# lyndonchan/wsss-analysis

Measured on AMD Instinct MI355X. Metric: images/sec CAM+CRF pseudo-labels, VOC2012 321x321, higher is better.
Workload: dtype f16x3; 1 GPU; resnet50 CAM + dense-CRF (M=21, 10 mean-field iters), 321x321, batch 32 images (=64 samples) per GPU, image-sharded; batch_images=32, num_classes=20, parallelism=image-sharded x1, no collective, steps_per_rank=239

## Files before the change

include/wsscam.h:

```cpp
#ifndef WSSCAM_H
#define WSSCAM_H

#include <stddef.h>
#include <stdint.h>

#ifdef __cplusplus
extern "C" {
#endif

#define WSC_VERSION 100

typedef enum wsc_status {
    WSC_OK = 0,
    WSC_ERR_INVALID = -1,
    WSC_ERR_NO_DEVICE = -2,
    WSC_ERR_HIP = -3,
    WSC_ERR_MISSING_KEY = -4,
    WSC_ERR_SHAPE = -5,
    WSC_ERR_NOMEM = -6,
    WSC_ERR_KEY_RANGE = -7,
    WSC_ERR_CAPACITY = -8,
    WSC_ERR_RANGE = -9
} wsc_status;

typedef enum wsc_arch {
    WSC_ARCH_RESNET50_CAM = 0,
    WSC_ARCH_VGG16_CAM = 1,
    WSC_ARCH_M7_CAM = 2,
    WSC_ARCH_RESNET50_IRN = 3,
    WSC_ARCH_VGG16_IRN = 4,
    WSC_ARCH_M7_IRN = 5,
    WSC_ARCH_DEEPLAB_LFOV = 6,
    WSC_ARCH_DEEPLAB_ASPP = 7
} wsc_arch;

typedef enum wsc_precision {
    WSC_PREC_BF16 = 0,
    WSC_PREC_BF16X3 = 1,
    WSC_PREC_F16 = 2,
    WSC_PREC_F16X3 = 3,
    WSC_PREC_F32 = 4
} wsc_precision;

typedef struct wsc_ctx wsc_ctx;
typedef struct wsc_net wsc_net;
typedef enum {
    WSC_OPT_CRF_GAUSS_ON_CHIP = 0,
    WSC_OPT_CRF_FUSED_BLUR = 1,
    WSC_OPT_CRF_BLUR_ON_CHIP = 2,
    WSC_OPT_CRF_RANK_BALLOT = 3,
    WSC_OPT_CRF_EMBED_FULL = 4,
    WSC_OPT_RW_TILED = 5,
    WSC_OPT_STEM_POOL_FUSED = 6,
    WSC_OPT_CONV_WINDOW = 7,
    WSC_OPT_CAM_HEAD_STREAM = 8,
    WSC_OPT_CRF_MSG_IN_UPDATE = 9,
    WSC_OPT_COUNT = 10
} wsc_option;

typedef struct wsc_crf wsc_crf;
typedef struct wsc_crf_v wsc_crf_v;

typedef struct wsc_tensor_desc {
    const char *name;
    const float *data;
    int32_t ndim;
    int64_t shape[4];
} wsc_tensor_desc;


int wsc_version(void);
const char *wsc_last_error(void);

int wsc_ctx_create(int device, void *stream, wsc_ctx **out);
void wsc_ctx_destroy(wsc_ctx *ctx);
int wsc_ctx_set_option(wsc_ctx *ctx, int option, int value);
int wsc_sync(wsc_ctx *ctx);
int wsc_ctx_range_status(wsc_ctx *ctx, int *flag_out, int clear);
int wsc_ctx_wait(wsc_ctx *ctx, wsc_ctx *other);
int wsc_ctx_mark(wsc_ctx *ctx, int slot);
int wsc_ctx_wait_mark(wsc_ctx *ctx, int slot);
int wsc_ctx_wait_for_mark(wsc_ctx *ctx, wsc_ctx *other, int slot);
int wsc_device_info(wsc_ctx *ctx, char *arch_name, size_t arch_name_len, int *num_cus);

int wsc_malloc(wsc_ctx *ctx, size_t bytes, void **dptr_out);
int wsc_free(wsc_ctx *ctx, void *dptr);
int wsc_memcpy_h2d(wsc_ctx *ctx, void *dst_dev, const void *src_host, size_t bytes);
int wsc_memcpy_d2h(wsc_ctx *ctx, void *dst_host, const void *src_dev, size_t bytes);
int wsc_memset(wsc_ctx *ctx, void *dst_dev, int value, size_t bytes);
int wsc_host_alloc(wsc_ctx *ctx, size_t bytes, void **host_out);
// ... 319 lines not shown
```

wsss-analysis_amd/csrc/common.h:

```cpp
#pragma once
#include <hip/hip_runtime.h>
#include <assert.h>
#include <stdint.h>
#include <map>
#include <string>
#include <unordered_map>
#include <vector>

#include "../../include/wsscam.h"

typedef uint16_t bf16_t;

typedef __bf16 bf16x8_t __attribute__((ext_vector_type(8)));
typedef _Float16 f16x8_t __attribute__((ext_vector_type(8)));
typedef float f32x16_t __attribute__((ext_vector_type(16)));
typedef float f32x4_t __attribute__((ext_vector_type(4)));

__host__ __device__ inline bf16_t f32_to_bf16(float f) {
    union { float f; uint32_t u; } v;
    v.f = f;
    uint32_t u = v.u;
    if ((u & 0x7fffffffu) > 0x7f800000u) return (bf16_t)((u >> 16) | 0x40);
    u += 0x7fffu + ((u >> 16) & 1u);
    return (bf16_t)(u >> 16);
// ... 85 lines not shown
    WSC_K_SLICE_UPDATE,
    WSC_K_CRF_MISC,
    WSC_K_WGRAD,
    WSC_K_GRAD_MISC,
    WSC_K_UPSAMPLE_GRAD,
    WSC_K_GN_GRAD,
    WSC_K_COUNT
};
struct WscProfRecord {
    int cls;
    double work;
    hipEvent_t e0, e1;
};

struct WscGaussCache;
void wsc_gauss_cache_destroy(WscGaussCache *cache);
struct wsc_ctx {
    int device = 0;
    hipStream_t stream = nullptr;
    bool own_stream = false;
    int num_cus = 0;
    std::string arch;
    void *ws = nullptr;
    size_t ws_bytes = 0;
    static constexpr int PIN_SLOTS = 8;
    struct PinSlot {
        void *p = nullptr;
        size_t bytes = 0;
        hipEvent_t ev = nullptr;
        bool busy = false;
    };
    PinSlot pin_ring[PIN_SLOTS];
    int pin_next = 0;
    int opt[WSC_OPT_COUNT] = {1, 1, 1, 0, 0, -1, 1, 1, 1, 1};
    void *zero_page = nullptr;
    unsigned *range_host = nullptr, *range_dev = nullptr;
    hipEvent_t ev0 = nullptr, ev1 = nullptr;
    hipEvent_t join_ev = nullptr;
    hipEvent_t marks[8] = {};
    bool mark_set[8] = {};
    hipStream_t aux_stream = nullptr;
    hipEvent_t fork_ev = nullptr, aux_done_ev = nullptr;
    bool profiling = false;
    std::vector<WscProfRecord> prof;
    std::vector<hipEvent_t> prof_pool;
    std::multimap<size_t, void *> free_blocks;
    std::unordered_map<void *, size_t> live_blocks;
    WscGaussCache *gauss_cache = nullptr;
};
int wsc_ctx_workspace(wsc_ctx *ctx, size_t bytes, void **out);
int wsc_ctx_range_check(wsc_ctx *ctx);
__device__ __forceinline__ unsigned half2_at_ceiling(unsigned hw) { return (hw & 0x7fff7fffu) + 0x04010401u; }
struct WscKernelTimer {
    wsc_ctx *ctx;
    int idx = -1;
    WscKernelTimer(wsc_ctx *c, int cls, double work);
    ~WscKernelTimer();
};
int wsc_ctx_cached_alloc(wsc_ctx *ctx, size_t bytes, void **out);
void wsc_ctx_cached_free(wsc_ctx *ctx, void *p);
struct WscCachedGuard {
    wsc_ctx *ctx;
    void *p;
    WscCachedGuard(wsc_ctx *c, void *q) : ctx(c), p(q) {}
    WscCachedGuard(const WscCachedGuard &) = delete;
    WscCachedGuard &operator=(const WscCachedGuard &) = delete;
    void free_now() {
// ... 334 lines not shown
```

wsss-analysis_amd/csrc/conv_igemm.hip:

```cpp
#include "common.h"

#include <type_traits>

namespace {

constexpr int BK = 64;

struct ConvKArgs {
    const bf16_t *x, *x_lo, *w;
    const float *s1, *b1, *s2, *b2;
    const bf16_t *res, *res_lo;
    bf16_t *y, *y_lo;
    float *y_f32;
    int H, W, Cin, Ho, Wo, Cout;
    int ldy;
    int kh, kw, stride, pad, relu;
    int M, HoWo;
    int m_base, m_end;
    unsigned div_howo_mul, div_howo_s1, div_howo_s2, div_wo_mul, div_wo_s1, div_wo_s2;
    int cchunks;
    int dil;
    int ksteps_base;
    int nk;
    int Kw;
    int Kbase;
    int ntiles_n, nblocks;
    const bf16_t *zero;
    int spare1;
    long long lo_delta;
    const bf16_t *x2;
    long long lo_delta2;
    int cc2, H2, W2, C2, stride2;
    int ldx;
    int win_npix;
    int spare2, spare3;
    unsigned *range;
};

__device__ __forceinline__ int lds_off(int row, int slot) {
    return row * 128 + ((slot ^ ((row >> 1) & 7)) << 4);
}

__device__ __forceinline__ void decode_row(const ConvKArgs &p, int m, int &n, int &ho, int &wo) {
    const unsigned t1 = __umulhi(p.div_howo_mul, (unsigned)m);
    n = (int)((t1 + (((unsigned)m - t1) >> p.div_howo_s1)) >> p.div_howo_s2);
    const int rem = m - n * p.HoWo;
    const unsigned t2 = __umulhi(p.div_wo_mul, (unsigned)rem);
    ho = (int)((t2 + (((unsigned)rem - t2) >> p.div_wo_s1)) >> p.div_wo_s2);
    wo = rem - ho * p.Wo;
}

template <int BM, int BN, int MODE, int SPLIT, int ET, int STAGES, int FAST = 0, int WPT = 0>
__global__ __launch_bounds__(BM * 2, (STAGES == 1 && FAST != 0) ? 4 : 2) void conv_igemm_kernel(ConvKArgs p) {
    constexpr bool GLDS = MODE == 0;
    constexpr int WMT = BM == 256 ? 128 : 64;
    constexpr bool FEPI = (FAST & 1) != 0, PW = (FAST & 2) != 0;
    constexpr bool WIN = WPT > 0;
    static_assert(!WIN || (SPLIT == 2 && BM == 128 && STAGES == 2 && FAST == 1), "LDS window: single-staged split, 128-row tile");
    static_assert(FAST == 0 || (SPLIT != 1 && ET == 1 && (MODE == 0 || FAST == 1)),
                  "FAST paths: f16, one plane or the single-staged split; the pointwise prologue belongs to the LDS-DMA layers");
    static_assert(SPLIT != 2 || (MODE == 0 && STAGES == 2), "single-staged split: LDS-DMA layers, two LDS buffers");
    static_assert(STAGES == 2 || SPLIT == 0, "one LDS buffer serves a one-K-step layer, which a layer of three K segments never is");
    constexpr int CK = SPLIT == 2 ? 32 : 64;
    constexpr int NT = BM * 2;
    constexpr int NW = BM / 32;
    constexpr int WR = BM / WMT;
    constexpr int WC = NW / WR;
    constexpr int WN = BN / WC;
    constexpr int MI = WMT / 32;
    constexpr int NI = WN / 32;
    static_assert(WR * WC == NW && WN % 32 == 0, "wave layout");
    constexpr int NB = BN * 8 / NT;
    constexpr int A_BYTES = BM * BK * 2;
    constexpr int B_BYTES = BN * BK * 2;
    constexpr int WIN_BYTES = WPT * 4096;
    constexpr int A_REGION = WIN ? WIN_BYTES : STAGES * A_BYTES;
    constexpr int CT_STRIDE = BN + 4;
    static_assert(GLDS || (BM == 128 && STAGES <= 2), "register staging exists for the 128-row tile only");
    static_assert(STAGES >= 1 && STAGES <= 2, "1 (single K-step layers) or 2 LDS buffers");

    extern __shared__ __attribute__((aligned(16))) char smem[];

    const int t = threadIdx.x;
    const int lane = t & 63;
    const int wv = __builtin_amdgcn_readfirstlane(t >> 6);
    const int wm = wv / WC, wn = wv - wm * WC;

    int tile;
    {
        const int bid = blockIdx.x;
// ... 103 lines not shown
                                                        c, 0, 0, 0);
        else
            c = __builtin_amdgcn_mfma_f32_32x32x16_f16(__builtin_bit_cast(f16x8_t, a), __builtin_bit_cast(f16x8_t, b),
                                                       c, 0, 0, 0);
    };
    auto mfma0 = [&](const u32x4_t &a, const u32x4_t &b) -> f32x16_t {
        const f32x16_t z = {0.f, 0.f, 0.f, 0.f, 0.f, 0.f, 0.f, 0.f, 0.f, 0.f, 0.f, 0.f, 0.f, 0.f, 0.f, 0.f};
        if (ET == 0)
            return __builtin_amdgcn_mfma_f32_32x32x16_bf16(__builtin_bit_cast(bf16x8_t, a), __builtin_bit_cast(bf16x8_t, b), z, 0, 0, 0);
        return __builtin_amdgcn_mfma_f32_32x32x16_f16(__builtin_bit_cast(f16x8_t, a), __builtin_bit_cast(f16x8_t, b), z, 0, 0, 0);
    };
    const unsigned lds0 = (unsigned)(uintptr_t)(__attribute__((address_space(3))) char *)smem;

    auto compute = [&](int buf) {
        const char *sa = smem + buf * A_BYTES;
        const char *sb = smem + STAGES * A_BYTES + buf * B_BYTES;
#pragma unroll
        for (int ks = 0; ks < 4; ++ks) {
            const int sl = ks * 2 + kgrp;
            u32x4_t af[MI], bfr[NI];
#pragma unroll
            for (int mi = 0; mi < MI; ++mi)
                af[mi] = *reinterpret_cast<const u32x4_t *>(sa + lds_off(wm * WMT + mi * 32 + l31, sl));
#pragma unroll
            for (int ni = 0; ni < NI; ++ni)
                bfr[ni] = *reinterpret_cast<const u32x4_t *>(sb + lds_off(wn * WN + ni * 32 + l31, sl));
#pragma unroll
            for (int mi = 0; mi < MI; ++mi)
#pragma unroll
                for (int ni = 0; ni < NI; ++ni) mfma(af[mi], bfr[ni], acc[mi][ni]);
        }
    };

    const int nk = STAGES == 1 ? 1 : p.nk;
    if (GLDS) {
        int n_seg = 0, n_khi = 0, n_kwi = 0, n_cc = 0, n_ktl = 0;
        const bf16_t *n_src = p.x;
        long long n_tap = 0;
        int n_wk = 0;
        auto prep = [&]() {
            n_src = (SPLIT == 1 && n_seg == 1) ? p.x_lo : p.x;
            if constexpr (FAST == 0) n_tap = ((long long)(n_khi * p.dil) * p.W + n_kwi * p.dil) * p.ldx + n_cc * CK;
            else n_tap = ((long long)n_khi * p.W + n_kwi) * p.ldx + n_cc * CK;
            if (SPLIT != 1 && p.x2 != nullptr && n_cc >= p.cc2) {
                n_src = p.x2;
                n_tap = (n_cc - p.cc2) * CK;
            }
            n_wk = ((SPLIT == 1 && n_seg == 2) ? p.Kbase : 0) + n_ktl * 64;
        };
        auto second_source = [&]() {
#pragma unroll
            for (int i = 0; i < 4; ++i) {
                const int m = m0 + lrow + RSTEP * i;
                int n, ho, wo;
                decode_row(p, m < p.m_end ? m : p.m_end - 1, n, ho, wo);
                const long long b2 = (((long long)n * p.H2 + ho * p.stride2) * p.W2 + wo * p.stride2) * (long long)p.C2;
                const int r = lrow + RSTEP * i;
                const int ks = slot ^ ((r >> 1) & 7);
                if (SPLIT == 2) aoff[i] = b2 + (ks & 3) * 8 + ((ks & 4) ? p.lo_delta2 : 0ll);
                else aoff[i] = b2 + ks * 8;
            }
        };
        auto advance = [&]() {
            ++n_ktl;
            if (++n_kwi == p.kw) {
                n_kwi = 0;
// ... 66 lines not shown
                const long long e = (long long)u * (long long)p.ldx + (sl & 3) * 8 + ((sl & 4) ? p.lo_delta : 0ll);
                woff[i] = ok ? (int)(e >> 3) : 0;
                wvalid |= ok ? (1u << i) : 0u;
            }
            win_load(0);
        }
        prep();
        if constexpr (!WIN) {
#pragma unroll
            for (int i = 0; i < 4; ++i) issue_a(i, 0);
        }
#pragma unroll
        for (int i = 0; i < NB; ++i) issue_b(i, 0);
        advance();
        if constexpr (WIN) win_store();
        if (ROLL && nk > 1) {
            prep();
#pragma unroll
            for (int i = 0; i < 4; ++i) issue_a(i, 1);
#pragma unroll
            for (int i = 0; i < NB; ++i) issue_b(i, 1);
            advance();
            asm volatile("s_waitcnt vmcnt(%0)" ::"n"(4 + NB) : "memory");
            __builtin_amdgcn_s_barrier();
        } else {
            __syncthreads();
        }
        unsigned offA[4], offB[4];
#pragma unroll
        for (int ks = 0; ks < 4; ++ks) {
            offA[ks] = lds0 + lds_off(wm * WMT + l31, ks * 2 + kgrp);
            offB[ks] = lds0 + A_REGION + lds_off(wn * WN + l31, ks * 2 + kgrp);
        }
        auto kstep = [&](auto cur_c, int kt) __attribute__((always_inline)) {
            constexpr int cur = decltype(cur_c)::value;
            const unsigned(&oA)[4] = offA, (&oB)[4] = offB;
            const bool more = kt + 1 < nk;
            if (more) {
                prep();
                if (SPLIT != 2) {
#pragma unroll
                    for (int i = 0; i < 4; ++i) issue_a(i, cur ^ 1);
#pragma unroll
                    for (int i = 0; i < NB; ++i) issue_b(i, cur ^ 1);
                }
            }
            if constexpr (SPLIT == 2) {
                u32x4_t fah[2][MI], fal[2][MI], fbh[2][NI], fbl[2][NI];
                constexpr int NAP = WIN ? 0 : 4;
                constexpr int EVERY = (6 * MI * NI) / (NAP + NB);
                static_assert(EVERY >= 1, "a K-step has room for every DMA piece");
                auto piece = [&](int j) {
                    if (!more || j % EVERY != 0) return;
                    const int q = j / EVERY;
                    if (q < NAP) issue_a(q, cur ^ 1);
                    else if (q < NAP + NB) issue_b(q - NAP, cur ^ 1);
                    __builtin_amdgcn_sched_barrier(0);
                };
                unsigned aw[MI][4];
                if constexpr (WIN) {
                    if ((c_khi | c_kwi) == 0 && c_cc + 1 < p.cchunks) win_load(c_cc + 1);
                    const int toff = c_khi * p.W + c_kwi;
                    const unsigned tbit = 1u << (c_khi * 3 + c_kwi);
#pragma unroll
                    for (int mi = 0; mi < MI; ++mi) {
                        const int pos = (tapmask[mi] & tbit) ? WIN_ZERO : qm[mi] + toff;
                        const unsigned b0 = lds0 + (unsigned)pos * 128u, sw = (unsigned)(pos >> 1) & 7u;
#pragma unroll
                        for (int pr = 0; pr < 4; ++pr) aw[mi][pr] = b0 + ((((unsigned)(pr * 2 + kgrp)) ^ sw) << 4);
                    }
                }
                auto rd = [&](int set, int sl) {
#pragma unroll
                    for (int mi = 0; mi < MI; ++mi) {
                        if constexpr (WIN) {
                            asm volatile("ds_read_b128 %0, %1" : "=v"(fah[set][mi]) : "v"(aw[mi][sl]) : "memory");
                            asm volatile("ds_read_b128 %0, %1" : "=v"(fal[set][mi]) : "v"(aw[mi][2 + sl]) : "memory");
                        } else {
                            asm volatile("ds_read_b128 %0, %1 offset:%2" : "=v"(fah[set][mi]) : "v"(oA[sl]), "n"(cur * A_BYTES + mi * 4096) : "memory");
                            asm volatile("ds_read_b128 %0, %1 offset:%2" : "=v"(fal[set][mi]) : "v"(oA[2 + sl]), "n"(cur * A_BYTES + mi * 4096) : "memory");
                        }
                    }
#pragma unroll
                    for (int ni = 0; ni < NI; ++ni) {
                        asm volatile("ds_read_b128 %0, %1 offset:%2" : "=v"(fbh[set][ni]) : "v"(oB[sl]), "n"(cur * B_BYTES + ni * 4096) : "memory");
                        asm volatile("ds_read_b128 %0, %1 offset:%2" : "=v"(fbl[set][ni]) : "v"(oB[2 + sl]), "n"(cur * B_BYTES + ni * 4096) : "memory");
                    }
                };
                rd(0, 0);
// ... 30 lines not shown
                }
            } else {
                u32x4_t fa[2][MI], fb[2][NI];

                auto rd = [&](int set, int ks) {
#pragma unroll
                    for (int mi = 0; mi < MI; ++mi)
                        asm volatile("ds_read_b128 %0, %1 offset:%2" : "=v"(fa[set][mi]) : "v"(oA[ks]), "n"(cur * A_BYTES + mi * 4096) : "memory");
#pragma unroll
                    for (int ni = 0; ni < NI; ++ni)
                        asm volatile("ds_read_b128 %0, %1 offset:%2" : "=v"(fb[set][ni]) : "v"(oB[ks]), "n"(cur * B_BYTES + ni * 4096) : "memory");
                };
                rd(0, 0);
#pragma unroll
                for (int ks = 0; ks < 4; ++ks) {
                    const int set = ks & 1;
                    if (ks < 3) {
                        rd(set ^ 1, ks + 1);
                        asm volatile("s_waitcnt lgkmcnt(%0)" ::"n"(MI + NI) : "memory");
                    } else {
                        asm volatile("s_waitcnt lgkmcnt(0)" ::: "memory");
                    }
                    __builtin_amdgcn_sched_barrier(0);
#pragma unroll
                    for (int mi = 0; mi < MI; ++mi)
#pragma unroll
                        for (int ni = 0; ni < NI; ++ni) {
                            if (STAGES == 1 && ks == 0) acc[mi][ni] = mfma0(fa[set][mi], fb[set][ni]);
                            else mfma(fa[set][mi], fb[set][ni], acc[mi][ni]);
                        }
                }
            }
            if (more) advance();
            __syncthreads();
            if constexpr (WIN) {
                if (++c_kwi == p.kw) {
                    c_kwi = 0;
                    if (++c_khi == p.kh) {
                        c_khi = 0;
                        ++c_cc;
                        if (more) {
                            win_store();
                            __syncthreads();
                        }
                    }
                }
            }
        };
        static_assert(A_BYTES + (MI - 1) * 4096 < 65536 && B_BYTES + (NI - 1) * 4096 < 65536, "ds_read immediate offset range");
        if constexpr (ROLL) {
            u32x4_t fah[MI], fal[MI], fbh[NI], fbl[NI];
            auto slice = [&](auto buf_c, auto pair_c, bool more, bool dma, int dbuf) __attribute__((always_inline)) {
                constexpr int nbuf = decltype(buf_c)::value, npair = decltype(pair_c)::value;
                const unsigned(&oA)[4] = offA, (&oB)[4] = offB;
                auto piece = [&](int j) {
                    if (!dma || j % 3 != 0) return;
                    const int q = j / 3;
                    if (q < 4) issue_a(q, dbuf);
                    else if (q < 4 + NB) issue_b(q - 4, dbuf);
                    __builtin_amdgcn_sched_barrier(0);
                };
                static_assert(3 * MI * NI >= 3 * (4 + NB), "a slice has room for every DMA piece");
                auto rdA = [&](u32x4_t(&f)[MI], int pair) {
#pragma unroll
                    for (int mi = 0; mi < MI; ++mi)
                        asm volatile("ds_read_b128 %0, %1 offset:%2" : "=v"(f[mi]) : "v"(oA[pair]), "n"(nbuf * A_BYTES + mi * 4096) : "memory");
                };
// ... 36 lines not shown
                        piece(2 * MI * NI + mi * NI + ni);
                    }
                __builtin_amdgcn_sched_barrier(0);
                if (more) {
                    rdB(fbh, npair);
                    rdA(fah, npair);
                }
            };
            {
                const unsigned(&oA)[4] = offA, (&oB)[4] = offB;
#pragma unroll
                for (int mi = 0; mi < MI; ++mi) asm volatile("ds_read_b128 %0, %1 offset:%2" : "=v"(fal[mi]) : "v"(oA[2]), "n"(mi * 4096) : "memory");
#pragma unroll
                for (int ni = 0; ni < NI; ++ni) asm volatile("ds_read_b128 %0, %1 offset:%2" : "=v"(fbl[ni]) : "v"(oB[2]), "n"(ni * 4096) : "memory");
#pragma unroll
                for (int ni = 0; ni < NI; ++ni) asm volatile("ds_read_b128 %0, %1 offset:%2" : "=v"(fbh[ni]) : "v"(oB[0]), "n"(ni * 4096) : "memory");
#pragma unroll
                for (int mi = 0; mi < MI; ++mi) asm volatile("ds_read_b128 %0, %1 offset:%2" : "=v"(fah[mi]) : "v"(oA[0]), "n"(mi * 4096) : "memory");
            }
            auto rstep = [&](auto cur_c, int kt) __attribute__((always_inline)) {
                constexpr int cur = decltype(cur_c)::value;
                slice(std::integral_constant<int, cur>{}, std::integral_constant<int, 1>{}, true, false, 0);
                __syncthreads();
                const bool refill = kt + 2 < nk;
                if (refill) prep();
                slice(std::integral_constant<int, cur ^ 1>{}, std::integral_constant<int, 0>{}, kt + 1 < nk, refill, cur);
                if (refill) advance();
            };
            for (int kt = 0; kt < nk; kt += 2) {
                rstep(std::integral_constant<int, 0>{}, kt);
                if (kt + 1 < nk) rstep(std::integral_constant<int, 1>{}, kt + 1);
            }
            __syncthreads();
        } else
        for (int kt = 0; kt < nk; kt += 2) {
            kstep(std::integral_constant<int, 0>{}, kt);
            if (kt + 1 < nk) kstep(std::integral_constant<int, 1>{}, kt + 1);
        }
    } else {
        load_tile(0);
        store_lds(0);
        __syncthreads();
        for (int kt = 0; kt < nk; ++kt) {
            const int cur = kt & 1;
            const bool more = kt + 1 < nk;
            if (more) load_tile(kt + 1);
            compute(cur);
            if (more) store_lds(cur ^ 1);
            __syncthreads();
        }
    }

    constexpr int TPR = BN / 8;
    constexpr int RPP = NT / TPR;
    constexpr int NPASS = BM / RPP;
    const int c8 = t % TPR;
    const int r0 = t / TPR;
    const int c = n0 + c8 * 8;
    const bool cok = c < p.Cout;
    const bool full = c + 8 <= p.Cout;
    const bool has_res = p.res != nullptr && full;
    constexpr bool PRE_ALL = WMT == 64 && !(STAGES == 1 && FEPI);
    constexpr int NHALF_R = STAGES == 1 ? BM / 64 : (WMT == 128 ? BM / 128 : 1);
    constexpr int NRES = PRE_ALL ? NPASS : NPASS / NHALF_R;
    uint4 rres[NRES], rres_lo[NRES];
    auto fetch_res = [&](int first_pass) {
#pragma unroll
        for (int i = 0; i < NRES; ++i) {
            const int m = m0 + (first_pass + i) * RPP + r0;
            rres[i] = make_uint4(0, 0, 0, 0);
            rres_lo[i] = make_uint4(0, 0, 0, 0);
            if (FEPI) {
                if (has_res) {
                    const int mc = m < p.m_end ? m : p.m_end - 1;
                    rres[i] = *reinterpret_cast<const uint4 *>(p.res + ((unsigned)mc * (unsigned)p.Cout + (unsigned)c));
                    if (SPLIT) rres_lo[i] = *reinterpret_cast<const uint4 *>(p.res_lo + ((unsigned)mc * (unsigned)p.Cout + (unsigned)c));
                }
            } else if (has_res && m < p.m_end) {
                const long long o = (long long)m * p.Cout + c;
                rres[i] = *reinterpret_cast<const uint4 *>(p.res + o);
                if (SPLIT) rres_lo[i] = *reinterpret_cast<const uint4 *>(p.res_lo + o);
            }
        }
    };
    if (PRE_ALL) fetch_res(0);
    const bool fpost = FEPI && p.s2 != nullptr;
    const float sat_lo = (p.relu && !fpost) ? 0.f : -65504.f;
    float s1[8], b1[8], s2[FEPI ? 1 : 8], b2[FEPI ? 1 : 8];
    const bool post = !FEPI && p.s2 != nullptr;
    if (FEPI) {
        const f32x4_t sa = *reinterpret_cast<const f32x4_t *>(p.s1 + c), sb = *reinterpret_cast<const f32x4_t *>(p.s1 + c + 4);
        const f32x4_t ba = *reinterpret_cast<const f32x4_t *>(p.b1 + c), bb = *reinterpret_cast<const f32x4_t *>(p.b1 + c + 4);
#pragma unroll
        for (int j = 0; j < 4; ++j) {
            s1[j] = sa[j];
            s1[4 + j] = sb[j];
            b1[j] = ba[j];
            b1[4 + j] = bb[j];
        }
    } else {
#pragma unroll
        for (int j = 0; j < 8; ++j) {
            s1[j] = cok ? p.s1[c + j] : 0.f;
            b1[j] = cok ? p.b1[c + j] : 0.f;
            s2[j] = (cok && post) ? p.s2[c + j] : 1.f;
            b2[j] = (cok && post) ? p.b2[c + j] : 0.f;
        }
    }

    float *ct = reinterpret_cast<float *>(smem);
    constexpr int NHALF = STAGES == 1 ? BM / 64 : (WMT == 128 ? BM / 128 : 1);
    constexpr int GR = BM / NHALF;
    constexpr int PPH = NPASS / NHALF;
    static_assert(NPASS % NHALF == 0 && PPH * RPP == GR && GR % WMT == 0, "epilogue pass layout");
    const int grp = (wm * WMT) / GR, roff = wm * WMT - grp * GR;
    unsigned ovf = 0u;
#pragma unroll
    for (int half = 0; half < NHALF; ++half) {
        if (half > 0) __syncthreads();
        if (!PRE_ALL) fetch_res(half * PPH);
        if (grp == half) {
#pragma unroll
            for (int mi = 0; mi < MI; ++mi)
#pragma unroll
                for (int ni = 0; ni < NI; ++ni)
#pragma unroll
                    for (int r = 0; r < 16; ++r) {
                        const int row = roff + mi * 32 + (r & 3) + 8 * (r >> 2) + 4 * kgrp;
                        const int col = wn * WN + ni * 32 + l31;
                        ct[row * CT_STRIDE + col] = acc[mi][ni][r];
                    }
        }
        __syncthreads();
        if (!cok) continue;
#pragma unroll
        for (int pp = 0; pp < PPH; ++pp) {
            const int pass = half * PPH + pp;
            const int lrow_e = pp * RPP + r0;
            const int m = m0 + half * GR + lrow_e;
            if (FEPI) {
// ... 99 lines not shown
                }
                if (p.y != nullptr && full) {
                    uint32_t hw[4], lw[4];
#pragma unroll
                    for (int j = 0; j < 4; ++j) {
                        const bf16_t h0 = f32_to_h16(v[2 * j], ET), h1 = f32_to_h16(v[2 * j + 1], ET);
                        hw[j] = (uint32_t)h0 | ((uint32_t)h1 << 16);
                        if (SPLIT) {
                            const float c0 = ET ? fminf(fmaxf(v[2 * j], -65504.f), 65504.f) : v[2 * j];
                            const float c1 = ET ? fminf(fmaxf(v[2 * j + 1], -65504.f), 65504.f) : v[2 * j + 1];
                            const bf16_t l0 = f32_to_h16(c0 - h16_to_f32(h0, ET), ET);
                            const bf16_t l1 = f32_to_h16(c1 - h16_to_f32(h1, ET), ET);
                            lw[j] = (uint32_t)l0 | ((uint32_t)l1 << 16);
                        }
                    }
                    if (ET) ovf |= half2_at_ceiling(hw[0]) | half2_at_ceiling(hw[1]) | half2_at_ceiling(hw[2]) | half2_at_ceiling(hw[3]);
                    const long long oy = (long long)m * p.ldy + c;
                    *reinterpret_cast<uint4 *>(p.y + oy) = make_uint4(hw[0], hw[1], hw[2], hw[3]);
                    if (SPLIT) *reinterpret_cast<uint4 *>(p.y_lo + oy) = make_uint4(lw[0], lw[1], lw[2], lw[3]);
                }
            }
        }
    }
    if (ET && (ovf & 0x80008000u)) *p.range = (unsigned)p.Cout;
}

typedef void (*ConvKernel)(ConvKArgs);
struct ConvVariant {
    ConvKernel kernel;
    int bm, bn;
    int lds;
    int cls;
};
template <int BM, int BN, int MODE, int SPLIT, int ET, int STAGES, int FAST = 0, int WPT = 0>
ConvVariant variant() {
    constexpr int A_BYTES = BM * BK * 2, B_BYTES = BN * BK * 2;
    constexpr int PIPE = WPT > 0 ? WPT * 4096 + STAGES * B_BYTES : STAGES * (A_BYTES + B_BYTES);
    constexpr int EPI = (STAGES == 1 ? 64 : (BM == 256 ? 128 : BM)) * (BN + 4) * 4;
    constexpr int LDS = PIPE > EPI ? PIPE : EPI;
    static_assert(LDS <= 160 * 1024, "LDS budget of a CU");
    return {conv_igemm_kernel<BM, BN, MODE, SPLIT, ET, STAGES, FAST, WPT>, BM, BN, LDS,
            MODE != 0 ? WSC_K_CONV_SMALLCIN : (BM == 256 ? WSC_K_CONV256 : (BN == 128 ? WSC_K_CONV128 : WSC_K_CONV64))};
}
template <int BM, int BN, int MODE, int ET, int FAST = 0>
ConvVariant one_plane(bool one_kstep) {
    if constexpr (BM == 128)
        if (one_kstep) return variant<BM, BN, MODE, 0, ET, 1, FAST>();
    return variant<BM, BN, MODE, 0, ET, 2, FAST>();
}
template <int BM, int BN>
ConvVariant select_variant(ConvForm form, wsc_precision prec, int fast, bool one_kstep, int wpt) {
    if constexpr (BM == 128) {
        auto small = [&](auto mode) {
            constexpr int MODE = decltype(mode)::value;
            switch (prec) {
            case WSC_PREC_BF16: return one_plane<128, BN, MODE, 0>(one_kstep);
            case WSC_PREC_BF16X3: return variant<128, BN, MODE, 1, 0, 2>();
            case WSC_PREC_F16: return fast ? one_plane<128, BN, MODE, 1, 1>(one_kstep) : one_plane<128, BN, MODE, 1>(one_kstep);
            default: return variant<128, BN, MODE, 1, 1, 2>();
            }
        };
        if (form == CONV_FORM_SMALL2) return small(std::integral_constant<int, 1>{});
        if (form == CONV_FORM_SMALL4) return small(std::integral_constant<int, 2>{});
        if (wpt == 8) return variant<128, BN, 0, 2, 1, 2, 1, 8>();
        if (wpt == 10) return variant<128, BN, 0, 2, 1, 2, 1, 10>();
    }
    ConvVariant v;
    switch (prec) {
    case WSC_PREC_BF16: v = one_plane<BM, BN, 0, 0>(one_kstep); break;
    case WSC_PREC_BF16X3: v = variant<BM, BN, 0, 1, 0, 2>(); break;
    case WSC_PREC_F16:
        v = fast == 3 ? one_plane<BM, BN, 0, 1, 3>(one_kstep) : (fast ? one_plane<BM, BN, 0, 1, 1>(one_kstep) : one_plane<BM, BN, 0, 1>(one_kstep));
        break;
    default:
        v = fast == 3 ? variant<BM, BN, 0, 2, 1, 2, 3>() : (fast ? variant<BM, BN, 0, 2, 1, 2, 1>() : variant<BM, BN, 0, 2, 1, 2>());
        break;
    }
    if (form == CONV_FORM_STEM_ROWS) v.cls = WSC_K_CONV_SMALLCIN;
    return v;
}
ConvVariant conv_variant(int bm, int bn, ConvForm form, wsc_precision prec, int fast, bool one_kstep, int wpt = 0) {
    if (bm == 256) return select_variant<256, 256>(form, prec, fast, one_kstep, wpt);
    return bn == 128 ? select_variant<128, 128>(form, prec, fast, one_kstep, wpt) : select_variant<128, 64>(form, prec, fast, one_kstep, wpt);
}

}

int conv_igemm_launch(wsc_ctx *ctx, const ConvLaunch &p) {
    if (p.prec == WSC_PREC_F32) return conv_f32_launch(ctx, p);
    WSC_CHECK(p.operands_match(), WSC_ERR_INVALID, "conv: an operand is not of the layer's precision %d", (int)p.prec);
    const int split = conv_split(p.prec), fmt = conv_fmt(p.prec);
    const bool dma = conv_form_dma(p.form);
    if (p.form == CONV_FORM_STEM_ROWS)
        WSC_CHECK(split == 2 && p.Cin == 4 && p.pad == 0 && p.kw <= 7 && (p.stride & 1) == 0, WSC_ERR_INVALID,
                  "conv: the padded-stem form needs split 2, a 4-channel padded input, kw <= 7 and an even stride");
    else if (p.form == CONV_FORM_GENERIC) WSC_CHECK(p.Cin % 64 == 0, WSC_ERR_INVALID, "conv: Cin=%d not a multiple of 64", p.Cin);
    else WSC_CHECK(p.Cin == 4, WSC_ERR_INVALID, "conv: small-Cin mode needs a 4-channel activation");
    const ConvKLayout k = conv_k_layout(p.kh, p.kw, p.Cin, p.form, p.prec);
    const bool single_staged = k.interleaved;
    ConvKArgs a = {};
    a.x = p.x.h16(); a.x_lo = p.x.h16_lo(); a.w = (const bf16_t *)p.w;
    a.s1 = p.s1; a.b1 = p.b1; a.s2 = p.s2; a.b2 = p.b2;
    a.res = p.res.h16(); a.res_lo = p.res.h16_lo();
    a.y = p.y.h16(); a.y_lo = p.y.h16_lo(); a.y_f32 = p.y_f32;
    a.H = p.H; a.W = p.W; a.Cin = p.Cin; a.Ho = p.Ho; a.Wo = p.Wo; a.Cout = p.Cout;
    a.ldy = p.ldy > 0 ? p.ldy : p.Cout;
    a.win_npix = 0;
    a.ldx = p.Cin; a.x2 = nullptr; a.lo_delta2 = 0; a.cc2 = 0; a.H2 = a.W2 = a.C2 = 0; a.stride2 = 1;
    a.kh = p.kh; a.kw = k.kw_steps; a.stride = p.stride; a.pad = p.pad; a.relu = p.relu;
    a.M = p.N * p.Ho * p.Wo;
    a.HoWo = p.Ho * p.Wo;
    conv_fastdiv((unsigned)(a.HoWo > 0 ? a.HoWo : 1), &a.div_howo_mul, &a.div_howo_s1, &a.div_howo_s2);
    conv_fastdiv((unsigned)(p.Wo > 0 ? p.Wo : 1), &a.div_wo_mul, &a.div_wo_s1, &a.div_wo_s2);
    WSC_CHECK(p.dil >= 1, WSC_ERR_INVALID, "conv: dilation %d", p.dil);
    const int dil = (p.kh == 1 && p.kw == 1) ? 1 : p.dil;
    WSC_CHECK(dil == 1 || (p.form == CONV_FORM_GENERIC && !p.x2), WSC_ERR_INVALID,
// ... 9 lines not shown
                  (!single_staged || p.x2.h16_lo() != nullptr),
                  WSC_ERR_INVALID, "conv: a second input needs a 1x1 / stride 1 layer, channel counts in multiples of 64 and no bf16x3");
        a.x2 = p.x2.h16();
        a.lo_delta2 = single_staged ? (long long)(p.x2.h16_lo() - a.x2) : 0;
        a.cc2 = K1 / k.ck;
        a.H2 = p.H2; a.W2 = p.W2; a.C2 = p.C2; a.stride2 = p.stride2;
        a.ldx = K1;
    }
    WSC_CHECK(p.CoutPad % 64 == 0, WSC_ERR_INVALID, "conv: CoutPad=%d not a multiple of 64", p.CoutPad);
    const int BN = conv_tile_bn(p.CoutPad);
    a.zero = (const bf16_t *)ctx->zero_page;
    a.range = ctx->range_dev;
    int fast = 0;
    if (!p.generic && dil == 1 && fmt && (split == 0 || single_staged) && p.y && p.y_f32 == nullptr &&
        p.Cout == p.CoutPad && (long long)a.M * a.ldy < (1ll << 31)) {
        fast = 1;
        if (dma && p.kh == 1 && p.kw == 1 && p.pad == 0 && p.stride == 1) fast = 3;
    }
    if (a.M == 0) return WSC_OK;
    auto launch = [&](const ConvVariant &v, int m_base, int m_end) -> int {
        ConvKArgs b = a;
        b.m_base = m_base;
        b.m_end = m_end;
        b.ntiles_n = p.CoutPad / v.bn;
        b.nblocks = ((m_end - m_base + v.bm - 1) / v.bm) * b.ntiles_n;
        WSC_TRY(wsc_set_max_dynamic_lds(ctx, reinterpret_cast<const void *>(v.kernel), v.lds));
        const double flops = 2.0 * (m_end - m_base) * a.Cout * (p.form == CONV_FORM_GENERIC ? (double)p.kh * p.kw * p.Cin : (double)p.kh * p.kw * 3);
        WscKernelTimer timer(ctx, v.cls, flops);
        hipLaunchKernelGGL(v.kernel, dim3(b.nblocks), dim3(v.bm * 2), v.lds, ctx->stream, b);
        WSC_HIP(hipGetLastError());
        return WSC_OK;
    };
    const bool one_kstep = a.nk == 1;
    const long long blocks_sq = ((a.M + 255) / 256) * (long long)(p.CoutPad / 256);
    bool square = dma && p.CoutPad % 256 == 0 && a.nk >= 4 && blocks_sq >= 192;
    if (split == 2 && !fast) square = false;
    if (split == 2 && a.nk < 16) square = false;
    if (square) {
        const ConvVariant sq = conv_variant(256, 256, p.form, p.prec, fast, one_kstep);
        const long long rounds = blocks_sq / ctx->num_cus, rem = blocks_sq - rounds * ctx->num_cus;
        if (rounds >= 1 && rem > 0 && rem * 2 <= ctx->num_cus && ctx->num_cus > 0) {
            const int big_rows = (int)((rounds * ctx->num_cus) / (p.CoutPad / 256));
            WSC_TRY(launch(sq, 0, big_rows * 256));
            return launch(conv_variant(128, BN, p.form, p.prec, fast, one_kstep), big_rows * 256, a.M);
        }
        return launch(sq, 0, a.M);
    }
    int wpt = 0;
    if (single_staged && fast == 1 && dil == 1 && p.kh == 3 && p.kw == 3 && p.stride == 1 && p.pad == 1 && !p.x2 &&
        p.Ho == p.H && p.Wo == p.W && ctx->opt[WSC_OPT_CONV_WINDOW] != 0) {
        const long long need = 127 + 2ll * p.W + 3 + 1;
        const long long npix = (long long)p.N * p.H * p.W;
        if (need <= 320 && npix < (1ll << 30) && a.lo_delta >= 0 && npix * p.Cin + a.lo_delta < (1ll << 33) && (a.lo_delta & 7) == 0) {
            a.win_npix = (int)npix;
            wpt = need <= 256 ? 8 : 10;
        }
    }
    return launch(conv_variant(128, BN, p.form, p.prec, fast, one_kstep, wpt), 0, a.M);
}
```

wsss-analysis_amd/wsscam/_lib.py:

```python
import ctypes
import os
import re
import threading

import numpy as np

_HERE = os.path.dirname(os.path.abspath(__file__))
LIB_PATH = os.path.join(_HERE, "libwsscam.so")
HEADER_PATH = os.path.normpath(os.path.join(_HERE, "..", "..", "include", "wsscam.h"))

WSC_OK = 0
WSC_ERR_INVALID = -1
WSC_ERR_NO_DEVICE = -2
WSC_ERR_HIP = -3
WSC_ERR_MISSING_KEY = -4
WSC_ERR_SHAPE = -5
WSC_ERR_NOMEM = -6
WSC_ERR_KEY_RANGE = -7
WSC_ERR_CAPACITY = -8
WSC_ERR_RANGE = -9

ARCH_RESNET50_CAM = 0
ARCH_VGG16_CAM = 1
ARCH_M7_CAM = 2
ARCH_RESNET50_IRN = 3
ARCH_VGG16_IRN = 4
ARCH_M7_IRN = 5
ARCH_DEEPLAB_LFOV = 6
ARCH_DEEPLAB_ASPP = 7

PREC_BF16 = 0
PREC_BF16X3 = 1
PREC_F16 = 2
PREC_F16X3 = 3
PREC_F32 = 4
OPT_CRF_GAUSS_ON_CHIP, OPT_CRF_FUSED_BLUR, OPT_CRF_BLUR_ON_CHIP, OPT_CRF_RANK_BALLOT, OPT_CRF_EMBED_FULL, OPT_RW_TILED, \
    OPT_STEM_POOL_FUSED, OPT_CONV_WINDOW, OPT_CAM_HEAD_STREAM, OPT_CRF_MSG_IN_UPDATE = range(10)
OPT_DEFAULTS = {OPT_CRF_GAUSS_ON_CHIP: 1, OPT_CRF_FUSED_BLUR: 1, OPT_CRF_BLUR_ON_CHIP: 1, OPT_CRF_RANK_BALLOT: 0,
                OPT_CRF_EMBED_FULL: 0, OPT_RW_TILED: -1, OPT_STEM_POOL_FUSED: 1, OPT_CONV_WINDOW: 1, OPT_CAM_HEAD_STREAM: 1,
                OPT_CRF_MSG_IN_UPDATE: 1}
CONV_GENERIC = 0x100


class WscError(RuntimeError):
    def __init__(self, status, message):
        super().__init__("libwsscam error %d: %s" % (status, message))
        self.status = status


class TensorDesc(ctypes.Structure):
    _fields_ = [
        ("name", ctypes.c_char_p),
        ("data", ctypes.POINTER(ctypes.c_float)),
        ("ndim", ctypes.c_int32),
        ("shape", ctypes.c_int64 * 4),
    ]


class TraceOp(ctypes.Structure):
    _fields_ = [(n, ctypes.c_int32) for n in (
        "kind", "in_", "in2", "res", "Ho", "Wo", "C", "coff", "pitch", "kh", "kw", "stride", "pad", "dil", "relu", "affine2", "stride2",
        "pool_rule", "pool_k", "pool_stride", "pool_pad", "pool_avg", "fused_next")] + [("label", ctypes.c_char * 100)]


class TapeEntry(ctypes.Structure):
    _fields_ = [("name", ctypes.c_char * 32), ("Ho", ctypes.c_int32), ("Wo", ctypes.c_int32), ("C", ctypes.c_int32),
                ("offset", ctypes.c_int64)]


class GradEntry(ctypes.Structure):
    _fields_ = [("name", ctypes.c_char * 32), ("kh", ctypes.c_int32), ("kw", ctypes.c_int32), ("Cin", ctypes.c_int32),
                ("Cout", ctypes.c_int32), ("w_off", ctypes.c_int64), ("b_off", ctypes.c_int64)]

# ... 1238 lines not shown
```

Measured before the change: 2620 images/s.

## Prefetch residual tile during final K-step of conv implicit GEMM

Adds a REARLY template variant of the LDS-DMA conv kernel that issues the residual-tensor loads for the epilogue during the second-to-last K-step. It peels the final two K-steps so it can wait on a precise vmcnt and place a raw barrier there. The goal is to hide residual-load latency behind the last MFMA steps instead of exposing it in the epilogue. The cost is extra VGPRs holding residual vectors through the main loop, which may reduce occupancy, and hand-written waitcnt encoding that must stay correct.

Result: no change. 2620 images/s (-0.0%).

```diff
diff --git a/include/wsscam.h b/include/wsscam.h
--- a/include/wsscam.h
+++ b/include/wsscam.h
@@ -55,7 +55,8 @@
     WSC_OPT_CONV_WINDOW = 7,
     WSC_OPT_CAM_HEAD_STREAM = 8,
     WSC_OPT_CRF_MSG_IN_UPDATE = 9,
-    WSC_OPT_COUNT = 10
+    WSC_OPT_CONV_RES_EARLY = 10,
+    WSC_OPT_COUNT = 11
 } wsc_option;
 
 typedef struct wsc_crf wsc_crf;
diff --git a/wsss-analysis_amd/csrc/common.h b/wsss-analysis_amd/csrc/common.h
--- a/wsss-analysis_amd/csrc/common.h
+++ b/wsss-analysis_amd/csrc/common.h
@@ -141,7 +141,7 @@
     };
     PinSlot pin_ring[PIN_SLOTS];
     int pin_next = 0;
-    int opt[WSC_OPT_COUNT] = {1, 1, 1, 0, 0, -1, 1, 1, 1, 1};
+    int opt[WSC_OPT_COUNT] = {1, 1, 1, 0, 0, -1, 1, 1, 1, 1, 1};
     void *zero_page = nullptr;
     unsigned *range_host = nullptr, *range_dev = nullptr;
     hipEvent_t ev0 = nullptr, ev1 = nullptr;
diff --git a/wsss-analysis_amd/csrc/conv_igemm.hip b/wsss-analysis_amd/csrc/conv_igemm.hip
--- a/wsss-analysis_amd/csrc/conv_igemm.hip
+++ b/wsss-analysis_amd/csrc/conv_igemm.hip
@@ -50,12 +50,14 @@
     wo = rem - ho * p.Wo;
 }
 
-template <int BM, int BN, int MODE, int SPLIT, int ET, int STAGES, int FAST = 0, int WPT = 0>
+template <int BM, int BN, int MODE, int SPLIT, int ET, int STAGES, int FAST = 0, int WPT = 0, int REARLY = 0>
 __global__ __launch_bounds__(BM * 2, (STAGES == 1 && FAST != 0) ? 4 : 2) void conv_igemm_kernel(ConvKArgs p) {
     constexpr bool GLDS = MODE == 0;
     constexpr int WMT = BM == 256 ? 128 : 64;
     constexpr bool FEPI = (FAST & 1) != 0, PW = (FAST & 2) != 0;
     constexpr bool WIN = WPT > 0;
+    static_assert(REARLY == 0 || (GLDS && BM == 128 && STAGES == 2 && FEPI && !WIN && SPLIT != 1),
+                  "early residual: 128-row LDS-DMA tiles with the FAST epilogue and two LDS buffers (launched with a residual and nk >= 2)");
     static_assert(!WIN || (SPLIT == 2 && BM == 128 && STAGES == 2 && FAST == 1), "LDS window: single-staged split, 128-row tile");
     static_assert(FAST == 0 || (SPLIT != 1 && ET == 1 && (MODE == 0 || FAST == 1)),
                   "FAST paths: f16, one plane or the single-staged split; the pointwise prologue belongs to the LDS-DMA layers");
@@ -225,6 +227,30 @@
         }
     };
 
+    constexpr int TPR = BN / 8;
+    constexpr int RPP = NT / TPR;
+    constexpr int NPASS = BM / RPP;
+    constexpr bool PRE_ALL = WMT == 64 && !(STAGES == 1 && FEPI);
+    constexpr int NHALF_R = STAGES == 1 ? BM / 64 : (WMT == 128 ? BM / 128 : 1);
+    constexpr int NRES = PRE_ALL ? NPASS : NPASS / NHALF_R;
+    static_assert(REARLY <= NRES, "early residual passes");
+    constexpr int NRL = REARLY * (SPLIT ? 2 : 1);
+    static_assert(NRL <= 32, "vmcnt is a 6-bit counter");
+    uint4 rres_e[REARLY > 0 ? REARLY : 1], rres_e_lo[REARLY > 0 ? REARLY : 1];
+    auto fetch_res_early = [&]() __attribute__((always_inline)) {
+        const unsigned cc = (unsigned)(n0 + (t % TPR) * 8);
+        const int rr = t / TPR;
+        __builtin_amdgcn_sched_barrier(0);
+#pragma unroll
+        for (int i = 0; i < REARLY; ++i) {
+            const int m = m0 + i * RPP + rr;
+            const int mc = m < p.m_end ? m : p.m_end - 1;
+            rres_e[i] = *reinterpret_cast<const uint4 *>(p.res + ((unsigned)mc * (unsigned)p.Cout + cc));
+            if (SPLIT) rres_e_lo[i] = *reinterpret_cast<const uint4 *>(p.res_lo + ((unsigned)mc * (unsigned)p.Cout + cc));
+        }
+        __builtin_amdgcn_sched_barrier(0);
+    };
+
     const int nk = STAGES == 1 ? 1 : p.nk;
     if (GLDS) {
         int n_seg = 0, n_khi = 0, n_kwi = 0, n_cc = 0, n_ktl = 0;
@@ -357,10 +383,10 @@
             offA[ks] = lds0 + lds_off(wm * WMT + l31, ks * 2 + kgrp);
             offB[ks] = lds0 + A_REGION + lds_off(wn * WN + l31, ks * 2 + kgrp);
         }
-        auto kstep = [&](auto cur_c, int kt) __attribute__((always_inline)) {
-            constexpr int cur = decltype(cur_c)::value;
+        auto kstep = [&](auto cur_c, auto ph_c, int kt) __attribute__((always_inline)) {
+            constexpr int cur = decltype(cur_c)::value, PH = decltype(ph_c)::value;
             const unsigned(&oA)[4] = offA, (&oB)[4] = offB;
-            const bool more = kt + 1 < nk;
+            const bool more = PH == 1 ? true : (PH == 2 ? false : kt + 1 < nk);
             if (more) {
                 prep();
                 if (SPLIT != 2) {
@@ -368,6 +394,7 @@
                     for (int i = 0; i < 4; ++i) issue_a(i, cur ^ 1);
 #pragma unroll
                     for (int i = 0; i < NB; ++i) issue_b(i, cur ^ 1);
+                    if constexpr (PH == 1) fetch_res_early();
                 }
             }
             if constexpr (SPLIT == 2) {
@@ -380,6 +407,8 @@
                     const int q = j / EVERY;
                     if (q < NAP) issue_a(q, cur ^ 1);
                     else if (q < NAP + NB) issue_b(q - NAP, cur ^ 1);
+                    if constexpr (PH == 1)
+                        if (q == NAP + NB - 1) fetch_res_early();
                     __builtin_amdgcn_sched_barrier(0);
                 };
                 unsigned aw[MI][4];
@@ -476,7 +505,12 @@
                 }
             }
             if (more) advance();
-            __syncthreads();
+            if constexpr (PH == 0) {
+                __syncthreads();
+            } else {
+                if constexpr (PH == 1) __builtin_amdgcn_s_waitcnt((NRL & 15) | (7 << 4) | (15 << 8) | ((NRL >> 4) << 14));
+                __builtin_amdgcn_s_barrier();
+            }
             if constexpr (WIN) {
                 if (++c_kwi == p.kw) {
                     c_kwi = 0;
@@ -579,10 +613,25 @@
                 if (kt + 1 < nk) rstep(std::integral_constant<int, 1>{}, kt + 1);
             }
             __syncthreads();
+        } else if constexpr (REARLY != 0) {
+            const std::integral_constant<int, 0> c0;
+            const std::integral_constant<int, 1> c1;
+            const std::integral_constant<int, 2> c2;
+            for (int kt = 0; kt + 2 < nk; kt += 2) {
+                kstep(c0, c0, kt);
+                if (kt + 3 < nk) kstep(c1, c0, kt + 1);
+            }
+            if (nk & 1) {
+                kstep(c1, c1, nk - 2);
+                kstep(c0, c2, nk - 1);
+            } else {
+                kstep(c0, c1, nk - 2);
+                kstep(c1, c2, nk - 1);
+            }
         } else
         for (int kt = 0; kt < nk; kt += 2) {
-            kstep(std::integral_constant<int, 0>{}, kt);
-            if (kt + 1 < nk) kstep(std::integral_constant<int, 1>{}, kt + 1);
+            kstep(std::integral_constant<int, 0>{}, std::integral_constant<int, 0>{}, kt);
+            if (kt + 1 < nk) kstep(std::integral_constant<int, 1>{}, std::integral_constant<int, 0>{}, kt + 1);
         }
     } else {
         load_tile(0);
@@ -598,23 +647,22 @@
         }
     }
 
-    constexpr int TPR = BN / 8;
-    constexpr int RPP = NT / TPR;
-    constexpr int NPASS = BM / RPP;
     const int c8 = t % TPR;
     const int r0 = t / TPR;
     const int c = n0 + c8 * 8;
     const bool cok = c < p.Cout;
     const bool full = c + 8 <= p.Cout;
-    const bool has_res = p.res != nullptr && full;
-    constexpr bool PRE_ALL = WMT == 64 && !(STAGES == 1 && FEPI);
-    constexpr int NHALF_R = STAGES == 1 ? BM / 64 : (WMT == 128 ? BM / 128 : 1);
-    constexpr int NRES = PRE_ALL ? NPASS : NPASS / NHALF_R;
+    const bool has_res = REARLY ? true : (p.res != nullptr && full);
     uint4 rres[NRES], rres_lo[NRES];
     auto fetch_res = [&](int first_pass) {
 #pragma unroll
         for (int i = 0; i < NRES; ++i) {
             const int m = m0 + (first_pass + i) * RPP + r0;
+            if (i < REARLY) {
+                rres[i] = rres_e[i];
+                rres_lo[i] = rres_e_lo[i];
+                continue;
+            }
             rres[i] = make_uint4(0, 0, 0, 0);
             rres_lo[i] = make_uint4(0, 0, 0, 0);
             if (FEPI) {
@@ -630,7 +678,7 @@
             }
         }
     };
-    if (PRE_ALL) fetch_res(0);
+    if (PRE_ALL && REARLY == 0) fetch_res(0);
     const bool fpost = FEPI && p.s2 != nullptr;
     const float sat_lo = (p.relu && !fpost) ? 0.f : -65504.f;
     float s1[8], b1[8], s2[FEPI ? 1 : 8], b2[FEPI ? 1 : 8];
@@ -653,6 +701,10 @@
             s2[j] = (cok && post) ? p.s2[c + j] : 1.f;
             b2[j] = (cok && post) ? p.b2[c + j] : 0.f;
         }
+    }
+    if constexpr (REARLY != 0) {
+        __builtin_amdgcn_sched_barrier(0);
+        fetch_res(0);
     }
 
     float *ct = reinterpret_cast<float *>(smem);
@@ -818,14 +870,14 @@
     int lds;
     int cls;
 };
-template <int BM, int BN, int MODE, int SPLIT, int ET, int STAGES, int FAST = 0, int WPT = 0>
+template <int BM, int BN, int MODE, int SPLIT, int ET, int STAGES, int FAST = 0, int WPT = 0, int REARLY = 0>
 ConvVariant variant() {
     constexpr int A_BYTES = BM * BK * 2, B_BYTES = BN * BK * 2;
     constexpr int PIPE = WPT > 0 ? WPT * 4096 + STAGES * B_BYTES : STAGES * (A_BYTES + B_BYTES);
     constexpr int EPI = (STAGES == 1 ? 64 : (BM == 256 ? 128 : BM)) * (BN + 4) * 4;
     constexpr int LDS = PIPE > EPI ? PIPE : EPI;
     static_assert(LDS <= 160 * 1024, "LDS budget of a CU");
-    return {conv_igemm_kernel<BM, BN, MODE, SPLIT, ET, STAGES, FAST, WPT>, BM, BN, LDS,
+    return {conv_igemm_kernel<BM, BN, MODE, SPLIT, ET, STAGES, FAST, WPT, REARLY>, BM, BN, LDS,
             MODE != 0 ? WSC_K_CONV_SMALLCIN : (BM == 256 ? WSC_K_CONV256 : (BN == 128 ? WSC_K_CONV128 : WSC_K_CONV64))};
 }
 template <int BM, int BN, int MODE, int ET, int FAST = 0>
@@ -835,7 +887,7 @@
     return variant<BM, BN, MODE, 0, ET, 2, FAST>();
 }
 template <int BM, int BN>
-ConvVariant select_variant(ConvForm form, wsc_precision prec, int fast, bool one_kstep, int wpt) {
+ConvVariant select_variant(ConvForm form, wsc_precision prec, int fast, bool one_kstep, int wpt, bool res_early) {
     if constexpr (BM == 128) {
         auto small = [&](auto mode) {
             constexpr int MODE = decltype(mode)::value;
@@ -850,6 +902,13 @@
         if (form == CONV_FORM_SMALL4) return small(std::integral_constant<int, 2>{});
         if (wpt == 8) return variant<128, BN, 0, 2, 1, 2, 1, 8>();
         if (wpt == 10) return variant<128, BN, 0, 2, 1, 2, 1, 10>();
+        if (res_early && form == CONV_FORM_GENERIC && fast && !one_kstep) {
+            constexpr int EALL = BN == 128 ? 8 : 4;
+            if (prec == WSC_PREC_F16) return fast == 3 ? variant<128, BN, 0, 0, 1, 2, 3, 0, EALL>() : variant<128, BN, 0, 0, 1, 2, 1, 0, EALL>();
+            if (prec == WSC_PREC_F16X3 && fast == 3) return variant<128, BN, 0, 2, 1, 2, 3, 0, 4>();
+            if constexpr (BN == 64)
+                if (prec == WSC_PREC_F16X3) return variant<128, 64, 0, 2, 1, 2, 1, 0, 4>();
+        }
     }
     ConvVariant v;
     switch (prec) {
@@ -865,9 +924,10 @@
     if (form == CONV_FORM_STEM_ROWS) v.cls = WSC_K_CONV_SMALLCIN;
     return v;
 }
-ConvVariant conv_variant(int bm, int bn, ConvForm form, wsc_precision prec, int fast, bool one_kstep, int wpt = 0) {
-    if (bm == 256) return select_variant<256, 256>(form, prec, fast, one_kstep, wpt);
-    return bn == 128 ? select_variant<128, 128>(form, prec, fast, one_kstep, wpt) : select_variant<128, 64>(form, prec, fast, one_kstep, wpt);
+ConvVariant conv_variant(int bm, int bn, ConvForm form, wsc_precision prec, int fast, bool one_kstep, int wpt = 0, bool res_early = false) {
+    if (bm == 256) return select_variant<256, 256>(form, prec, fast, one_kstep, wpt, false);
+    return bn == 128 ? select_variant<128, 128>(form, prec, fast, one_kstep, wpt, res_early)
+                     : select_variant<128, 64>(form, prec, fast, one_kstep, wpt, res_early);
 }
 
 }
@@ -943,6 +1003,7 @@
         return WSC_OK;
     };
     const bool one_kstep = a.nk == 1;
+    const bool res_early = ctx->opt[WSC_OPT_CONV_RES_EARLY] != 0 && a.res != nullptr && fast != 0 && dma && a.nk >= 2;
     const long long blocks_sq = ((a.M + 255) / 256) * (long long)(p.CoutPad / 256);
     bool square = dma && p.CoutPad % 256 == 0 && a.nk >= 4 && blocks_sq >= 192;
     if (split == 2 && !fast) square = false;
@@ -953,7 +1014,7 @@
         if (rounds >= 1 && rem > 0 && rem * 2 <= ctx->num_cus && ctx->num_cus > 0) {
             const int big_rows = (int)((rounds * ctx->num_cus) / (p.CoutPad / 256));
             WSC_TRY(launch(sq, 0, big_rows * 256));
-            return launch(conv_variant(128, BN, p.form, p.prec, fast, one_kstep), big_rows * 256, a.M);
+            return launch(conv_variant(128, BN, p.form, p.prec, fast, one_kstep, 0, res_early), big_rows * 256, a.M);
         }
         return launch(sq, 0, a.M);
     }
@@ -967,5 +1028,5 @@
             wpt = need <= 256 ? 8 : 10;
         }
     }
-    return launch(conv_variant(128, BN, p.form, p.prec, fast, one_kstep, wpt), 0, a.M);
+    return launch(conv_variant(128, BN, p.form, p.prec, fast, one_kstep, wpt, res_early), 0, a.M);
 }
diff --git a/wsss-analysis_amd/wsscam/_lib.py b/wsss-analysis_amd/wsscam/_lib.py
--- a/wsss-analysis_amd/wsscam/_lib.py
+++ b/wsss-analysis_amd/wsscam/_lib.py
@@ -35,10 +35,10 @@
 PREC_F16X3 = 3
 PREC_F32 = 4
 OPT_CRF_GAUSS_ON_CHIP, OPT_CRF_FUSED_BLUR, OPT_CRF_BLUR_ON_CHIP, OPT_CRF_RANK_BALLOT, OPT_CRF_EMBED_FULL, OPT_RW_TILED, \
-    OPT_STEM_POOL_FUSED, OPT_CONV_WINDOW, OPT_CAM_HEAD_STREAM, OPT_CRF_MSG_IN_UPDATE = range(10)
+    OPT_STEM_POOL_FUSED, OPT_CONV_WINDOW, OPT_CAM_HEAD_STREAM, OPT_CRF_MSG_IN_UPDATE, OPT_CONV_RES_EARLY = range(11)
 OPT_DEFAULTS = {OPT_CRF_GAUSS_ON_CHIP: 1, OPT_CRF_FUSED_BLUR: 1, OPT_CRF_BLUR_ON_CHIP: 1, OPT_CRF_RANK_BALLOT: 0,
                 OPT_CRF_EMBED_FULL: 0, OPT_RW_TILED: -1, OPT_STEM_POOL_FUSED: 1, OPT_CONV_WINDOW: 1, OPT_CAM_HEAD_STREAM: 1,
-                OPT_CRF_MSG_IN_UPDATE: 1}
+                OPT_CRF_MSG_IN_UPDATE: 1, OPT_CONV_RES_EARLY: 1}
 CONV_GENERIC = 0x100
 
 
```
